# HongjianFang/DSurfTomo

Hardware: AMD Instinct MI355X
Metric: source-period FMM solves/sec on NxN grid; travel-time max-abs-err vs ref (higher is better)
Workload: dtype f32

## Files before the change

dsurftomo_amd/csrc/bundle_kernel.hip:

```cpp
#include "kernels.h"
#include "receiver_core.h"
#include "wave_ops.h"

namespace dsa {

namespace {

__device__ __forceinline__ unsigned bf2u(float f) { return __float_as_uint(f); }
__device__ __forceinline__ float bu2f(unsigned u) { return __uint_as_float(u); }

enum { BC_READY = 0, BC_READY_ODD, BC_TMIN, BC_THETA, BC_FREEZE, BC_HASH, BC_OVERFLOW, BC_CUR, BC_STALE, BC_STALEMIN, BC_SLOWN, BC_FARALL, BC_COUNT };
constexpr int kFarStrikes = 8;
constexpr int kBundleCycleRounds = 8;
constexpr float kStaleWindows = 16.0f;
constexpr int kStaleRounds = 6;

typedef __attribute__((address_space(1))) unsigned long long BGU64;
typedef __attribute__((address_space(1))) char BGChar;
typedef __attribute__((address_space(1))) float BGF32;
typedef __attribute__((address_space(1))) const float BGCF32;
typedef float __attribute__((ext_vector_type(4))) BV4;
typedef __attribute__((address_space(1))) BV4 BGV4;
typedef float __attribute__((ext_vector_type(2))) BV2;
template <int MPL> struct BMem;
template <> struct BMem<4> { typedef BV4 V; typedef __attribute__((address_space(1))) BV4 GV; };
template <> struct BMem<2> { typedef BV2 V; typedef __attribute__((address_space(1))) BV2 GV; };
// ... 17 lines not shown
template <int CH>
__device__ __forceinline__ unsigned node_or(unsigned v)
{
    if (CH >= 2) v |= (unsigned)__builtin_amdgcn_update_dpp(0, (int)v, 0xb1, 0xf, 0xf, false);
    if (CH >= 4) v |= (unsigned)__builtin_amdgcn_update_dpp(0, (int)v, 0x4e, 0xf, 0xf, false);
    if (CH >= 8) v |= (unsigned)__builtin_amdgcn_update_dpp(0, (int)v, 0x141, 0xf, 0xf, false);
    return v;
}

}

#ifdef DSA_BUNDLE_WAVES
#define DSA_BUNDLE_OCC(G, NT, MPL) __attribute__((amdgpu_waves_per_eu(DSA_BUNDLE_WAVES, DSA_BUNDLE_WAVES)))
#else
#define DSA_BUNDLE_OCC(G, NT, MPL) __attribute__((amdgpu_waves_per_eu((((NT) == 256 && ((MPL) == 2 || (G) == 16)) || (NT) == 768) ? 3 : 1, (((NT) == 256 && ((MPL) == 2 || (G) == 16)) || (NT) == 768) ? 3 : 2)))
#endif
template <int G, int NT, int MPL = 4, bool TIE = false>
__global__ __launch_bounds__(NT) DSA_BUNDLE_OCC(G, NT, MPL) void k_fim_bundle(const FimBundle* __restrict__ bundles, const FimProblem* __restrict__ problems,
                                                    const FimEnds* __restrict__ ends)
{
    constexpr int NW = NT / 64;
    constexpr int CH = G / MPL;
    typedef typename BMem<MPL>::V BV;
    typedef typename BMem<MPL>::GV BGV;
    constexpr int NPW = 64 / CH;
    constexpr unsigned GB = G * 4u * DSA_BSTRIDE;
    extern __shared__ unsigned dyn_lds[];
    __shared__ int sc[BC_COUNT];
    constexpr int kWaveBuf = 256, kTileBuf = NT > 256 ? 128 : 256, kClrWords = 4;
    __shared__ int wbuf[NW * kWaveBuf];
// ... 81 lines not shown
    BGChar* const Pb = (BGChar*)(Bslot + bd->p_offset);
    auto pv = [&](int id) -> float { return *(BGF32*)(Pb + ((unsigned)id << 2)); };

    __syncthreads();
    bool dead = false;
    {
        const BV4 inf4 = { kInf, kInf, kInf, kInf };
        for (int i = tid; i < ntile * (kTileRecs * G / 4) * DSA_BSTRIDE; i += NT) ((BGV4*)Bb)[i] = inf4;
        for (int i = tid; i < ntile * (kTileRecs / 4); i += NT) ((BGV4*)Pb)[i] = inf4;
        for (int i = tid; i < (1 << xlog); i += NT) *exc_at((unsigned)i) = kExcEmpty;
        for (int i = tid; i < (ntile << (kMaskShift - 3)); i += NT) *(BGU64*)(maskb + ((size_t)i << 3)) = 0ull;
        for (int i = tid; i < nwords; i += NT) tb[i] = 0u;
        if (tid == 0) {
            sc[BC_READY] = 0; sc[BC_READY_ODD] = 0; sc[BC_TMIN] = 0x7f800000; sc[BC_THETA] = 0x7f800000;
            sc[BC_FREEZE] = (int)0xff800000u; sc[BC_HASH] = 0; sc[BC_OVERFLOW] = 0; sc[BC_CUR] = 0; sc[BC_STALE] = (int)0xff800000u; sc[BC_STALEMIN] = 0x7f800000;
            sc[BC_SLOWN] = 0; sc[BC_FARALL] = bd->far_all ? 1 : 0;
            if (TIE && bd->cand) *(bd->cand + (size_t)my_slot * bd->cand_stride) = 0;
        }
        if (TIE && bd->cand) {
            BGV4* const seen4 = (BGV4*)(bd->cand + (size_t)my_slot * bd->cand_stride + ((bd->cand_cap + 4) & ~3));
            const BV4 zero4 = { 0.0f, 0.0f, 0.0f, 0.0f };
            for (int i = tid; i < kTieSeenSlots / 4; i += NT) seen4[i] = zero4;
        }
        __threadfence_block();
        __syncthreads();
        typedef __attribute__((address_space(1))) const Rec GCRec;
        for (int m = 0; m < nmem; ++m) {
            const FimEnds* const E = ends + s_member[m];
            const FimProblem* const pm = problems + s_member[m];
            const bool from_records = E->Fpin != nullptr;
            GCRec* const W = from_records ? (GCRec*)E->Fpin : (GCRec*)E->W;
// ... 60 lines not shown
        h.in[1] = ix + 1 < nnx;    h.in_outer[1] = ix + 2 < nnx;
        h.in[2] = iz > 0;          h.in_outer[2] = iz > 1;
        h.in[3] = iz + 1 < nnz;    h.in_outer[3] = iz + 2 < nnz;
        float val[9], tau[9];
        int kid[9];
#pragma unroll
        for (int q = 0; q < 4; ++q) {
            val[q] = h.in[q] ? *(BGF32*)(Bb + (unsigned)nid[q] * GB + mb) : kInf;
            val[4 + q] = h.in_outer[q] ? *(BGF32*)(Bb + (unsigned)nid[4 + q] * GB + mb) : kInf;
            kid[q] = nid[q]; kid[4 + q] = nid[4 + q];
        }
        val[8] = *(BGF32*)(Bb + (unsigned)id * GB + mb);
        kid[8] = id;
#pragma unroll
        for (int q = 0; q < 9; ++q) tau[q] = val[q];
#pragma nounroll
        for (int it = 0; it < 9; ++it) {
            float v = val[0], t = tau[0];
            if (__builtin_signbit(v)) { bool pin; t = exc_lookup(kid[0] * G + mo, &pin); v = pin ? v : -v; }
            const int k0 = kid[0];
#pragma unroll
            for (int j = 0; j < 8; ++j) { val[j] = val[j + 1]; tau[j] = tau[j + 1]; kid[j] = kid[j + 1]; }
            val[8] = v; tau[8] = t; kid[8] = k0;
        }
#pragma unroll
        for (int q = 0; q < 4; ++q) { h.near_[q] = val[q]; h.near_tau[q] = tau[q]; h.outer[q] = val[4 + q]; h.outer_tau[q] = tau[4 + q]; }
        *t_old = val[8]; *k_old = tau[8];
    };
    auto slow_member = [&](int id, int mo, int half, float stale, unsigned& evals, unsigned& nchanged, unsigned& hv_lane, float& kmin_lane, float& smin_lane) -> bool {
        if (mo >= nmem) return false;
// ... 61 lines not shown
        float t_old, k_old;
        load_hood(id, mo, ix, iz, h, &t_old, &k_old);
        if (t_pinned(t_old)) return;
        float k = kInf, ti = -1.0f;
        const float slown = *(BGCF32*)(slowb + (unsigned)id * npb + (unsigned)s_map[mo] * 4u);
        const NodeGeom geom = { p.ri, risti[ix], p.dnx, p.dnz };
        (void)solve_node_t<true>(h, slown, geom, &k, &ti);
        const FimProblem* const pm = problems + s_member[mo];
        if (ti >= 0.0f && pm->tie) {
            if (ti > 0.0f) { atomicAdd((unsigned*)pm->tie + 2, 1u); atomicAdd((unsigned*)pm->tie + 3, (unsigned)(fminf(ti, 1.0f) * (1.0f / kTieSumUnit))); }
            else atomicAdd((unsigned*)pm->tie + 5, 1u);
            if (ti > pm->tie_threshold) { atomicAdd((unsigned*)pm->tie, 1u); atomicMax((unsigned*)pm->tie + 1, bf2u(ti)); }
        }
    };
    int* const wq = slowq + wave * kSlowQ;
    int qn = 0;
    int cn = 0;
    int* const cand_g = (TIE && bd->cand && bd->cand_list) ? bd->cand + (size_t)my_slot * bd->cand_stride : nullptr;
    const bool listing = TIE && __builtin_amdgcn_readfirstlane(cand_g != nullptr ? 1 : 0) != 0;
    bool clost = false;
    auto cand_push = [&](bool on, int word) {
        const unsigned long long bal = __ballot(on);
        if (!bal) return;
        const int pos = cn + __popcll(bal & ((1ull << lane) - 1ull));
        cn += __popcll(bal);
        if (qn + cn >= kSlowQ - 1) { clost = true; return; }
        if (on) wq[kSlowQ - 1 - pos] = word;
    };
    auto cand_flush = [&]() {
        if (!cn || !cand_g) { cn = 0; clost = false; return; }
        int base = -1;
        if (lane == 0) {
            if (clost) (void)atomicMax(cand_g, bd->cand_cap + 1);
            else if (__hip_atomic_load(cand_g, __ATOMIC_RELAXED, __HIP_MEMORY_SCOPE_AGENT) <= bd->cand_cap) base = atomicAdd(cand_g, cn);
        }
        base = __builtin_amdgcn_readfirstlane(base);
        if (!clost && base >= 0) for (int i = lane; i < cn; i += 64) if (base + i < bd->cand_cap) cand_g[1 + base + i] = wq[kSlowQ - 1 - i];
        cn = 0; clost = false;
    };

    int rounds = 0, stall = 0, freezes = 0, sm_same = 0, far_strikes = 0;
    float sm_prev = kInf, sm_prev2 = kInf;
    unsigned hist[4] = { 1u, 2u, 3u, 4u };
    float best_tmin = -kInf;
    unsigned evals = 0, nchanged = 0;
    const int sub = lane % CH, nslot = lane / CH;
    const unsigned sub_b = (unsigned)sub * (4u * MPL);
    unsigned mp[MPL], vmask = 0u;
#pragma unroll
    for (int m = 0; m < MPL; ++m) { mp[m] = (unsigned)s_map[sub * MPL + m] * 4u; if (sub * MPL + m < nmem) vmask |= 1u << m; }
    bool sl_vec = (bd->np % MPL) == 0;
    {
        const int base = sub * MPL < nmem ? s_map[sub * MPL] : 0;
        sl_vec = sl_vec && (base % MPL) == 0 && base + MPL <= bd->np;
#pragma unroll
        for (int m = 1; m < MPL; ++m) if (sub * MPL + m < nmem && s_map[sub * MPL + m] != base + m) sl_vec = false;
        if (sl_vec) mp[0] = (unsigned)base * 4u;
    }
    sl_vec = __all(sl_vec);

#ifdef DSA_BUNDLE_CLOCKS
    unsigned long long bt[4] = { 0, 0, 0, 0 }, bt0 = wall_clock64();
#define DSA_BCLK(k) do { const unsigned long long t1_ = wall_clock64(); bt[k] += t1_ - bt0; bt0 = t1_; } while (0)
#else
#define DSA_BCLK(k) do { } while (0)
#endif
    for (; !dead;) {
        const float theta = bu2f((unsigned)sc[BC_THETA]);
        const bool open = !(theta < kInf);
        const float freeze = bu2f((unsigned)sc[BC_FREEZE]);
        const bool frozen_any = freeze > -kInf;
        const float stale = bu2f((unsigned)sc[BC_STALE]);
        const float far_margin = sc[BC_FARALL] ? kInf : far_margin0;

        int seen = 0;
        float tmin_lane = kInf;
        int* const nbuf = wbuf + wave * kWaveBuf;
        int* const tbuf = wtile + wave * kTileBuf;
        unsigned* const clr = wclr + wave * kTileBuf * kClrWords;
        constexpr int kQ = kTileBuf / 64, kI = kWaveBuf / 64;
// ... 150 lines not shown
                        if (idx >= tbase && idx < tbase + take) tbuf[ntw + idx - tbase] = (w << 5) + b2;
                        ++idx;
                    }
                    ntw += take; tbase += take;
                }
                if (ntw) { sweep_tiles(ntw); ntw = 0; }
            }
        }
        tmin_lane = wave_min(tmin_lane);
        if (lane == 0) {
            if (tmin_lane < kInf) atomicMin(reinterpret_cast<unsigned*>(&sc[BC_TMIN]), bf2u(tmin_lane));
            if (seen) atomicAdd(&sc[BC_CUR], seen);
        }
        __syncthreads();
        DSA_BCLK(0);
        const int cnt = sc[BC_CUR];
        if (cnt == 0) break;

        const int nready_even = sc[BC_READY] < rhalf ? sc[BC_READY] : rhalf;
        const int nready_odd = sc[BC_READY_ODD] < rhalf ? sc[BC_READY_ODD] : rhalf;
        unsigned hv_lane = 0u;
        float kmin_lane = kInf, smin_lane = kInf;
        for (int half = 0; half < 2; ++half) {
            const int nready = half ? nready_odd : nready_even;
            for (int j0 = wave * NPW; j0 < nready; j0 += NW * NPW) {
                const int j = j0 + nslot;
                const bool act = j < nready;
                const unsigned ent = act ? (unsigned)ready[half ? rhalf + j : j] : 0u;
                const int id = (int)(ent & ((1u << kFarShift) - 1u));
                const unsigned farc = ent >> kFarShift;
// ... 74 lines not shown
                __builtin_amdgcn_s_setprio(1);
                if (any_changed) {
                    *(BGV*)(Bb + (unsigned)id * GB + sub_b) = outv;
                    if (sub == 0) *(BGF32*)(Pb + ((unsigned)id << 2)) = outv[0];
                }
                bool any_slow = false;
#pragma unroll
                for (int m = 0; m < MPL; ++m) any_slow = any_slow | slowm[m];
                if (__any(any_slow)) {
                    bool again = false;
#pragma unroll
                    for (int m = 0; m < MPL; ++m) {
                        const bool push = slowm[m];
                        const unsigned long long bal = __ballot(push);
                        const int pos = qn + __popcll(bal & ((1ull << lane) - 1ull));
                        if (push && pos < kSlowQ - 1 - cn) wq[pos] = (id << 4) | (sub * MPL + m);
                        again = again || (push && pos >= kSlowQ - 1 - cn);
                        qn += __popcll(bal);
                    }
                    if (again) { atomicOr((unsigned long long*)(mask_at(id >> 6) + half), 1ull << (id & 63)); atomicOr(&tb[(id >> 6) >> 5], 1u << ((id >> 6) & 31)); }
                }
                if (listing) {
                    unsigned tiem = 0u;
#pragma unroll
                    for (int m = 0; m < MPL; ++m) {
                        const float v = outv[m];
                        const bool eq = (v == vn[0][m]) | (v == vn[1][m]) | (v == vn[2][m]) | (v == vn[3][m]);
                        tiem |= (eq & (v < kInf) & donem[m]) ? 1u << m : 0u;
                    }
                    if (__any(tiem != 0u)) {
#pragma nounroll
                        for (int m = 0; m < MPL; ++m) cand_push(((tiem >> m) & 1u) != 0u, (id << 4) | (sub * MPL + m));
                    }
                }
                unsigned wm = 0u;
#pragma unroll
                for (int q = 0; q < 4; ++q) wm |= (actn[q] ? 1u << q : 0u) | ((acto[q] & in_outer[q]) ? 16u << q : 0u);
                wm = node_or<CH>(wm);
                {
                    const unsigned chg = node_or<CH>(any_changed ? 1u : 0u);
                    const float pt = outv[0];
                    if (sub == 0 && chg && !__builtin_signbit(pt) && pt < stale) smin_lane = fminf(smin_lane, pt);
                }
                if (sub == 0 && wm) activate_node(id, wm, half);
            }
            if (lane == 0 && qn) atomicAdd(&sc[BC_SLOWN], qn);
            qn = qn < kSlowQ - 1 - cn ? qn : max(kSlowQ - 1 - cn, 0);
            for (int base = 0; base < qn; base += 64) {
                const int e = base + lane < qn ? wq[base + lane] : -1;
                bool tied = false;
                if (e >= 0) tied = slow_member(e >> 4, e & 15, half, stale, evals, nchanged, hv_lane, kmin_lane, smin_lane);
                if (listing) cand_push(tied, (int)((unsigned)e | kCandAlways));
            }
            qn = 0;
            if (TIE) cand_flush();
            if (half == 1) {
                const unsigned hv = wave_sum(hv_lane);
                const float kmin = wave_min(kmin_lane), smin = wave_min(smin_lane);
                if (lane == 0) {
                    if (hv) atomicAdd(reinterpret_cast<unsigned*>(&sc[BC_HASH]), hv);
                    if (kmin < kInf) atomicMin(reinterpret_cast<unsigned*>(&sc[BC_TMIN]), bf2u(kmin));
                    if (smin < kInf) atomicMin(reinterpret_cast<unsigned*>(&sc[BC_STALEMIN]), bf2u(smin));
                }
            }
            __syncthreads();
            DSA_BCLK(1 + half);
        }
        if (tid == 0) {
            {
                const int slown = sc[BC_SLOWN];
                sc[BC_SLOWN] = 0;
                if (!sc[BC_FARALL]) {
                    if (slown * 12 > (nready_even + nready_odd) * nmem && nready_even + nready_odd >= 64) { if (++far_strikes >= kFarStrikes) sc[BC_FARALL] = 1; }
                    else if (far_strikes > 0) --far_strikes;
                }
            }
            sc[BC_READY] = 0; sc[BC_READY_ODD] = 0; sc[BC_CUR] = 0;
            float tmin = bu2f((unsigned)sc[BC_TMIN]);
            {
                const float sm = bu2f((unsigned)sc[BC_STALEMIN]);
                sc[BC_STALEMIN] = 0x7f800000;
// ... 9 lines not shown
            sc[BC_STALE] = (int)bf2u(best_tmin - kStaleWindows * p.window);
            const bool repeat = hsh != 0u && (hsh == hist[1] || hsh == hist[2] || hsh == hist[3] || hsh == hist[0]);
            hist[3] = hist[2]; hist[2] = hist[1]; hist[1] = hist[0]; hist[0] = hsh;
            if (repeat) { if (++stall >= kBundleCycleRounds) { const float fz = (sm_same >= kStaleRounds ? sm_prev : best_tmin) + p.window;
                                                                 if (fz > bu2f((unsigned)sc[BC_FREEZE])) sc[BC_FREEZE] = (int)bf2u(fz); stall = 0; ++freezes; } }
            else stall = 0;
        }
        ++rounds;
        __syncthreads();
        DSA_BCLK(3);
        if (sc[BC_OVERFLOW]) break;
        if (rounds > p.max_rounds) { dead = true; break; }
    }
    const bool failed = rounds > p.max_rounds;
#ifdef DSA_BUNDLE_CLOCKS
    if (tid == 0 && p.clocks) { p.clocks[0] = bt[0]; p.clocks[1] = bt[1]; p.clocks[2] = bt[2]; p.clocks[3] = bt[3]; }
#endif

    {
        unsigned long long e64 = evals, c64 = nchanged;
        for (int o = 32; o > 0; o >>= 1) { e64 += __shfl_xor(e64, o); c64 += __shfl_xor(c64, o); }
        if (lane == 0) { atomicAdd(reinterpret_cast<unsigned long long*>(p.info + 4), e64); atomicAdd(reinterpret_cast<unsigned long long*>(p.info + 6), c64); }
    }
    __threadfence_block();
    __syncthreads();
    if (TIE && !failed && !sc[BC_OVERFLOW]) {
        constexpr int LPN = G / 4, NPI = 64 / LPN;
        const int csub = lane % LPN, cnode = lane / LPN;
        const BV4 inf4 = { kInf, kInf, kInf, kInf };
        int cq = 0;
        bool lost = false;
// ... 170 lines not shown
                    }
                }
            }
        }
        census_flush();
        if (lost && lane < nmem) {
            const FimProblem* const pm = problems + s_member[lane];
            if (pm->tie) { atomicAdd((unsigned*)pm->tie, 1u); atomicMax((unsigned*)pm->tie + 1, bf2u(kInf)); }
        }
        __syncthreads();
    }
    for (int m = 0; m < nmem; ++m) {
        const FimEnds* const E = ends + s_member[m];
        const FimProblem* const pm = problems + s_member[m];
        if (tid == 0) {
            pm->info[0] = rounds; pm->info[1] = 0; pm->info[3] = m == 0 ? freezes : 0;
            if (TIE && pm->tie) { pm->tie[4] = freezes; pm->tie[7] = cand_g ? __hip_atomic_load(cand_g, __ATOMIC_RELAXED, __HIP_MEMORY_SCOPE_AGENT) : -1; }
            if (failed && pm->info[2] != -2) pm->info[2] = -1;
            if (sc[BC_OVERFLOW]) pm->info[2] = -2;
        }
        if (E->rays) {
            const GridDesc g = E->g;
            for (int r = tid; r < E->nrays; r += NT) {
                const RayDesc rd = E->rays[r];
                if (!(rd.flags & kRayTime)) continue;
                float t;
                if (!receiver_time(g, E->scx, E->scz, rd, (const float*)Bslot + m, E->veln, E->dpl, &t, G * DSA_BSTRIDE)) atomicExch(E->err, E->ray0 + r + 1);
                E->out[rd.data] = t;
            }
        }
    }
// ... 111 lines not shown
```

dsurftomo_amd/csrc/engine.h:

```cpp
#pragma once

#include <hip/hip_runtime.h>

#include <string>
#include <vector>

#include "host_geometry.h"
#include "kernels.h"

namespace dsa {

template <class T>
struct DevBuf {
    T* p = nullptr;
    size_t cap = 0;
};

struct SpmvState;

constexpr int kDefaultExactTies = 1;
constexpr float kDefaultTieThreshold = 2.0e-5f;
constexpr float kDefaultTieSumThreshold = 0.0f;
constexpr int kDefaultTieCountThreshold = 0;
constexpr int kDefaultTieFrozenBundles = 0;
// ... 56 lines not shown
    int field_pool_opt = 0;
    size_t per_slot_bytes = 0;
    size_t plan_budget = 0;
    std::vector<int> h_launch_rank;
    int bundle_opt = 1;
    int ray_lanes_opt = 0;
    float bundle_window_opt = 0.0f;
    int bundle_G_now = 0;
    int bundle_threads_opt = 0;
    int bundle_max_rounds = 0;
    int bundle_mpl = 0;
    bool bundle_wide = false;
    int bundle_mpl_now = 4, bundle_mpl_b = 2;
    int bundle_threads_b = 256;
    int bundle_tail_opt = 1;
    int bundle_far_all = 0;
    int bundles_a = 0, bundles_b = 0, bundle_Gb = 0;
    hipStream_t stream2 = nullptr;
    hipEvent_t ev_b0 = nullptr, ev_b1 = nullptr;
    hipError_t make_stream2();
    int bundle_refined_opt = 1;
    bool refined_bundles_failed = false;
    bool refined_bundles_now = false;
    std::vector<FimBundle> h_bundles_r;
    DevBuf<FimBundle> bundles_r_d;
    DevBuf<FimEnds> ends_r;
    DevBuf<float> Br_pool, slowIr;
    DevBuf<unsigned long long> exc_br;
    DevBuf<int> lists_br, cand_br;
    size_t slowIr_off_b = 0;
// ... 156 lines not shown
```

dsurftomo_amd/csrc/engine.hip:

```cpp
#include <hip/hip_runtime.h>

#include <algorithm>
#include <chrono>
#include <cstdarg>
#include <cstdio>
#include <cstring>
#include <string>
#include <map>
#include <vector>

#include "../../include/dsurftomo_amd.h"
#include "engine.h"

namespace dsa {

static std::string g_create_error;

void Engine::fail(int code, const char* fmt, ...)
{
    char buf[512];
    va_list ap;
    va_start(ap, fmt);
    vsnprintf(buf, sizeof buf, fmt, ap);
    va_end(ap);
// ... 817 lines not shown
            stats[DSA_STAT_BUNDLES] += nbundles; stats[DSA_STAT_BUNDLED_UNITS] += n - nsolo;
            stats[DSA_STAT_FOOTPRINT_MB] = std::max(stats[DSA_STAT_FOOTPRINT_MB], ((double)pool_slots * (double)per_slot_bytes + (double)chunk * (double)per_unit_bytes) / 1.0e6 + bundle_mb);
        }
        for (int u = 0; u < n; ++u) {
            const int32_t* fi = &h_info[(size_t)u * 16];
            if (fi[10] == -3) { fail(DSA_ERR_INTERNAL, "unit %d: no free field slot within the wait bound (pool of %d slots, claimed by compare-and-swap: a pool smaller than the resident workgroups on very long solves, or corrupted busy flags; set option field_pool = -1 for a slot per unit)", first + u, pool_slots); return DSA_ERR_INTERNAL; }
            if (fi[2] < 0 || fi[10] == -1) { fail(DSA_ERR_INTERNAL, "unit %d: fixed-point solve did not converge (rounds %d/%d)", first + u, fi[0], fi[8]); return DSA_ERR_INTERNAL; }
            if (h_flags[(size_t)u * 4 + 1]) { fail(DSA_ERR_INTERNAL, "unit %d: serial march guard %d (1/17 window, 2/18 tree, 32 exception table)", first + u, h_flags[(size_t)u * 4 + 1]); return DSA_ERR_INTERNAL; }
            stats[DSA_STAT_ROUNDS_MAX] = std::max(stats[DSA_STAT_ROUNDS_MAX], (double)fi[8]);
            h_unit_rounds[(size_t)(first + u)] = fi[8];
            unsigned long long ev;
            std::memcpy(&ev, fi + 12, 8);
            stats[DSA_STAT_EVALS_TOTAL] += (double)ev;
            std::memcpy(&ev, fi + 14, 8);
            stats[DSA_STAT_CHANGES_TOTAL] += (double)ev;
            stats[DSA_STAT_RESCANS] += fi[1] + fi[9];
            stats[DSA_STAT_FREEZES] += fi[3] + fi[11];
        }
        if (!h_tie0.empty()) {
            const std::vector<char> fl = tie_verdicts(first, n, h_tie0.data(), h_info.data(), nbundles > 0);
            for (int u = 0; u < n; ++u) if (fl[(size_t)u]) { h_unit_flags[(size_t)(first + u)] |= 1; stats[DSA_STAT_TIE_UNITS] += 1.0; stats[DSA_STAT_TIE_UNITS_LEFT] += 1.0; }
        }
        for (int u = 0; u < n; ++u) stats[DSA_STAT_TIE_INFLUENCE_MAX] = std::max(stats[DSA_STAT_TIE_INFLUENCE_MAX], (double)h_unit_tie[(size_t)(first + u)]);
        last_chunk_first = first;
        last_chunk_n = n;
        fields_resident = n <= pool_slots && !marched_in_tiles;
        if (rows && trace_chunk(first, n, rw, iw, col, cap, nar) != 0) return status;
      } while (redo_chunk);
    }
    HIP_TRY(this, hipEventRecord(events[7], stream));
    HIP_TRY(this, hipEventSynchronize(events[7]));
// ... 188 lines not shown
    if (want_cand && ensure(cand_b, slots_total * cand_stride)) return status;
    if (ensure(B_pool, b_total) || ensure(exc_b, exc_total) || ensure(lists_b, slots_total * lists_c_stride) || ensure(bpool_gen, slots_total) ||
        ensure(bundles_d, (size_t)nb) || ensure(member_flag, (size_t)n) || ensure(slowI, (size_t)nmaps * nrec_c)) return status;
    if (!slowI_ready) { launch_interleave_maps(slow.p, nrec_c, nmaps, slowI.p, stream); slowI_ready = true; }
    h_bundles.assign((size_t)nb, FimBundle{});
    int rank = nsolo;
    for (int k = 0; k < nb; ++k) {
        const Group& r = gr[k < bundles_a ? 0 : 1];
        const std::vector<int>& mem = k < bundles_a ? pieces[(size_t)k].second : tail[(size_t)(k - bundles_a)].second;
        const int kk = k < bundles_a ? k : k - bundles_a;
        FimBundle& bd = h_bundles[(size_t)k];
        bd.B = B_pool.p + r.b_off; bd.b_stride = r.b_stride; bd.p_offset = (size_t)r.G * DSA_BSTRIDE * nrec_c;
        bd.exc = exc_b.p + r.exc_off; bd.exc_stride = (size_t)1 << r.xlog; bd.exc_log2cap = r.xlog;
        bd.lists = lists_b.p + r.slot0 * lists_c_stride; bd.lists_stride = lists_c_stride;
        bd.slot_busy = r.slots < r.count ? bpool_gen.p + r.slot0 : nullptr; bd.nslots = r.slots; bd.slot = r.slots < r.count ? 0 : kk;
        bd.slowI = slowI.p; bd.np = nmaps; bd.far_all = bundle_far_all;
        bd.cand = want_cand ? cand_b.p + r.slot0 * cand_stride : nullptr; bd.cand_stride = cand_stride; bd.cand_cap = (int)cand_cap; bd.cand_list = tie_list_opt;
        bd.nmem = (int)mem.size();
        for (int m = 0; m < kBundleMax; ++m) { bd.member[m] = 0; bd.map[m] = 0; }
        for (int m = 0; m < bd.nmem; ++m) {
            const int u = mem[(size_t)m];
            h_launch_rank[(size_t)u] = rank;
            bd.member[m] = rank++;
            bd.map[m] = h_src[(size_t)(first + u)].period;
        }
    }
    refined_bundles_now = bundle_refined_opt && (nb >= 128 || bundle_refined_opt == 2) && !refined_bundles_failed && exact_ties != 2;
    if (refined_bundles_now) {
        const size_t nrec_r = kRefRecs;
        const int xlog_r0 = exc_log2cap_of(kRefMax, kRefMax);
        const size_t lists_r_stride = ((size_t)kFimMaskInts * kRefTiles * kRefTiles + 2 + 1) & ~(size_t)1;
// ... 375 lines not shown
    if (n == "fim_sorted" && (value == 0 || value == 1)) { en->planned = false; en->fim_sorted = (int)value; return 0; }
    if (n == "ray_path_cap" && value >= 0 && value <= (1 << 24)) { en->ray_path_cap = (int)value; return 0; }
    if (n == "disp_group_shift" && value >= -1 && value <= 3) { en->disp_group_shift = (int)value; return 0; }
    if (n == "disp_layers_lds" && (value == -1 || value == 0 || value == 1)) { en->disp_layers_lds = (int)value; return 0; }
    if (n == "exc_log2cap" && (value == 0 || (value >= 6 && value <= 24))) { en->planned = false; en->exc_log2cap_opt = (int)value; return 0; }
    if (n == "rows_on_device" && (value == 0 || value == 1)) { en->rows_on_device = value != 0; return 0; }
    if (n == "lsmr_device_vectors" && (value == 0 || value == 1)) { en->lsmr_device_vectors = (int)value; return 0; }
    if (n == "field_pool" && value >= -1) { en->planned = false; en->field_pool_opt = (int)value; return 0; }
    if (n == "ray_lanes" && (value == 0 || value == 1 || value == 4)) { en->ray_lanes_opt = (int)value; return 0; }
    if (n == "bundle_window_cells" && value >= 0) { en->bundle_window_opt = (float)value; return 0; }
    if (n == "bundle_threads" && (value == 0 || value == 256 || value == 512 || value == 768)) { en->bundle_threads_opt = (int)value; return 0; }
    if (n == "bundle_max_rounds" && value >= 0) { en->bundle_max_rounds = (int)value; return 0; }
    if (n == "bundle_tail" && (value == 0 || value == 1)) { en->bundle_tail_opt = (int)value; return 0; }
    if (n == "bundle_refined" && (value == 0 || value == 1 || value == 2)) { en->bundle_refined_opt = (int)value; return 0; }
    if (n == "bundle_far_all" && (value == 0 || value == 1)) { en->bundle_far_all = (int)value; return 0; }
    if (n == "bundle_pool" && value >= 0) { en->bundle_pool_opt = (int)value; return 0; }
    if (n == "bundle_members_per_lane" && (value == 0 || value == 4 || value == 2)) { en->bundle_mpl = (int)value; return 0; }
    if (n == "bundle" && (value == 0 || value == 1 || value == 4 || value == 8 || value == 16)) { en->planned = false; en->bundle_opt = (int)value; return 0; }
    if (n == "exact_ties" && (value == 0 || value == 1 || value == 2)) { en->exact_ties = (int)value; return 0; }
    if (n == "tie_threshold" && value >= 0) { en->tie_threshold = (float)value; return 0; }
    if (n == "tie_detect" && (value == 0 || value == 1)) { en->tie_detect = (int)value; return 0; }
    if (n == "tie_sum_threshold" && value >= 0) { en->tie_sum_threshold = (float)value; return 0; }
    if (n == "tie_count_threshold" && value >= 0) { en->tie_count_threshold = (int)value; return 0; }
    if (n == "tie_frozen_bundles" && (value == 0 || value == 1)) { en->tie_frozen_bundles = (int)value; return 0; }
    if (n == "tie_map_strict" && (value == 0 || value == 1)) { en->tie_map_strict = (int)value; return 0; }
    if (n == "tie_scale_guard" && (value == 0 || value == 1)) { en->tie_scale_guard = (int)value; return 0; }
    if (n == "handoff_replay" && (value == 0 || value == 1)) { en->handoff_replay = (int)value; return 0; }
    if (n == "tie_tolerance" && value > 0) { en->tie_tolerance = (float)value; return 0; }
    if (n == "bundle_order" && (value == 0 || value == 1 || value == 2 || value == 3)) { en->bundle_order_opt = (int)value; return 0; }
    if (n == "tie_list" && (value == 0 || value == 1)) { en->tie_list_opt = (int)value; return 0; }
// ... 260 lines not shown
```

dsurftomo_amd/csrc/kernels.h:

```cpp
#pragma once

#include <hip/hip_runtime.h>
#include <stdint.h>

#include "source_stage.h"

namespace dsa {

struct RayDesc { int src; float rx, rz; float sin_rx; int data; int flags; };
constexpr int kRayTime = 1, kRayPath = 2;

constexpr int kClockSlots = 32;
constexpr int kTieWords = 16;
constexpr float kTieSumUnit = 0x1p-30f;
constexpr int kTieSeenLog2 = 14, kTieSeenSlots = 1 << kTieSeenLog2;

struct FimProblem {
    Rec* F;
    float* Tc;
    unsigned long long* exc;
    int exc_log2cap;
    const float* slow;
    const float* risti;
    const int* seed;
// ... 59 lines not shown
    unsigned long long* exc;
    size_t exc_stride;
    int exc_log2cap;
    int* lists;
    size_t lists_stride;
    size_t p_offset;
    int* slot_busy;
    int nslots, slot;
    const float* slowI;
    int np;
    int* cand;
    size_t cand_stride;
    int cand_cap;
    int cand_list;
    int far_all;
    int nmem;
    int member[kBundleMax];
    int map[kBundleMax];
};
size_t bundle_lds_bytes(int tile_words);
void launch_fim_bundles(const FimBundle* d_bundles, int nbundles, int G, int threads , const FimProblem* d_problems, const FimEnds* d_ends, int tile_words, hipStream_t stream,
                        int members_per_lane = 4 ,
                        bool tie = false );
void launch_interleave_maps(const float* d_slow_all, size_t field_stride, int np, float* d_slowI, hipStream_t stream);

size_t fim_lds_bytes(const FimLaunch& l);
void launch_fim(const FimProblem* d_problems, int nproblems, const FimLaunch& l, hipStream_t stream, const FimEnds* d_ends = nullptr);

void launch_gridder(const GridDesc& g, const float* d_velv, const float* d_basis, float* d_veln, float* d_slow,
                    hipStream_t stream);
// ... 100 lines not shown
```

dsurftomo_amd/csrc/stage_kernels.hip:

```cpp
#include "kernels.h"
#include "receiver_core.h"
#include "exact_march.h"

namespace dsa {

namespace {

__device__ __forceinline__ SourceScratch scratch_of(const BatchPtrs& b, int s)
{
    SourceScratch w;
    const size_t rr = (size_t)kRefMax * kRefMax;
    w.slow_r = b.slow_r + (size_t)s * kRefRecs;
    w.F_r = b.F_r + (size_t)s * kRefRecs;
    w.S_r = b.S_r + s * rr;
    w.risti_r = b.risti_r + (size_t)s * kRefMax;
    w.vcorner = b.vcorner + (size_t)s * 4;
    w.rst = b.rst + (size_t)s * kRWin * kRWin;
    w.cst = b.cst + (size_t)s * kCWinMax * kCWinMax;
    w.cinit = b.cinit + (size_t)s * kCWinMax * kCWinMax;
    w.heap = b.heap + (size_t)s * kHeapCap;
    w.flags = b.flags + (size_t)s * 4;
    return w;
}

// ... 394 lines not shown
                                const float* risti_c, float window_r, float window_c, FimProblem* prob_r,
                                FimProblem* prob_c, int32_t* info, unsigned long long* clocks, const int* __restrict__ launch_rank,
                                int32_t* tie, float tie_threshold, FimEnds* ends_c, const RayDesc* __restrict__ rays, const float* __restrict__ veln_all,
                                size_t veln_stride, float dpl, float* out, int32_t* err, const int* __restrict__ member_flag, float window_b, int max_rounds_b, float window_t, FimEnds* ends_r)
{
    const int s = blockIdx.x * blockDim.x + threadIdx.x;
    if (s >= nsrc) return;
    const SourceDesc sd = b.src[s];
    FimProblem r;
    r.Tc = nullptr; r.exc = nullptr; r.exc_log2cap = 0;
    r.F = b.F_r + (size_t)s * kRefRecs; r.slow = b.slow_r + (size_t)s * kRefRecs; r.risti = b.risti_r + (size_t)s * kRefMax;
    r.seed = b.seed_r + (size_t)s * kSeedR; r.seed_count = b.nseed_r + s; r.seed_cap = kSeedR; r.lists = b.lists + (size_t)s * b.lists_stride;
    r.nnx = sd.rnx; r.nnz = sd.rnz; r.nbx = sd.nbx_r; r.nbz = sd.nbz_r;
    r.ri = g.earth; r.dnx = sd.rdnx; r.dnz = sd.rdnz; r.window = window_r;
    r.max_rounds = 64 * (sd.rnx + sd.rnz) + 4096;
    r.clocks = nullptr;
    r.info = info + (size_t)s * 16;
    r.tie = tie ? tie + (size_t)s * kTieWords : nullptr; r.tie_threshold = tie_threshold;
    r.ended = b.flags + (size_t)s * 4;
    const int rank = launch_rank ? launch_rank[s] : s;
    if (ends_r) {
        prob_r[rank] = r;
        FimEnds er{};
        er.Fpin = r.F;
        ends_r[rank] = er;
    } else prob_r[s] = r;
    const bool recycled = b.pool < nsrc;
    const int slot = recycled ? rank % b.pool : s;
    const bool member = member_flag && member_flag[s];
    FimProblem c;
    c.F = nullptr;
// ... 67 lines not shown
```

dsurftomo_amd/engine.py:

```python
import ctypes as C
import os

import numpy as np

_HERE = os.path.dirname(os.path.abspath(__file__))
LIB_PATH = os.environ.get("DSA_LIB_PATH") or os.path.join(_HERE, "libdsurftomo_amd.so")

STAT_NAMES = ("ms_total", "ms_fim_coarse", "ms_fim_refined", "ms_stages", "launches_fim_coarse", "units",
              "rounds_max", "evals_total", "chunk", "rescans", "freezes", "rays", "ray_steps", "rays_clamped",
              "ms_rays", "ms_rows", "nar", "ms_dispersion", "curves", "changes_total", "tie_units", "exact_units", "exact_pops", "ms_exact", "field_slots", "footprint_mb", "bundle_size", "bundles", "bundled_units", "bundle_slots", "bundle_threads", "tie_units_left", "tie_influence_max", "exact_pool", "exact_tiles", "tie_units_strict", "tie_prone_maps", "tie_units_tied", "tie_units_by_scale", "handoffs_replayed")

_f32, _i32, _vp = C.c_float, C.c_int, C.c_void_p
_lib = None


class EngineError(RuntimeError):
    def __init__(self, code, text):
        super().__init__("dsurftomo_amd error %d: %s" % (code, text))
        self.code = code


def load_library():
    global _lib
    if _lib is not None:
        return _lib
# ... 408 lines not shown
```

include/dsurftomo_amd.h:

```cpp
#ifndef DSURFTOMO_AMD_H
#define DSURFTOMO_AMD_H

#include <stddef.h>
#include <stdint.h>

#ifdef __cplusplus
extern "C" {
#endif

typedef struct dsa_engine dsa_engine;

enum dsa_status {
    DSA_OK = 0,
    DSA_ERR_DEVICE = -1,
    DSA_ERR_ARGUMENT = -2,
    DSA_ERR_OUTSIDE = -3,
    DSA_ERR_INTERNAL = -4,
    DSA_ERR_STATE = -5,
    DSA_ERR_CAPACITY = -6
};

int dsa_create(dsa_engine** out, int device_index);
void dsa_destroy(dsa_engine* e);
const char* dsa_error_string(const dsa_engine* e);
// ... 96 lines not shown
       DSA_STAT_LAUNCHES_FIM_COARSE, DSA_STAT_UNITS, DSA_STAT_ROUNDS_MAX, DSA_STAT_EVALS_TOTAL,
       DSA_STAT_CHUNK, DSA_STAT_RESCANS, DSA_STAT_FREEZES, DSA_STAT_RAYS, DSA_STAT_RAY_STEPS,
       DSA_STAT_RAYS_CLAMPED, DSA_STAT_MS_RAYS, DSA_STAT_MS_ROWS, DSA_STAT_NAR, DSA_STAT_MS_DISPERSION,
       DSA_STAT_CURVES, DSA_STAT_CHANGES_TOTAL, DSA_STAT_TIE_UNITS, DSA_STAT_EXACT_UNITS, DSA_STAT_EXACT_POPS,
       DSA_STAT_MS_EXACT, DSA_STAT_FIELD_SLOTS, DSA_STAT_FOOTPRINT_MB, DSA_STAT_BUNDLE_SIZE, DSA_STAT_BUNDLES,
       DSA_STAT_BUNDLED_UNITS, DSA_STAT_BUNDLE_SLOTS, DSA_STAT_BUNDLE_THREADS,
       DSA_STAT_TIE_UNITS_LEFT,
       DSA_STAT_TIE_INFLUENCE_MAX,
       DSA_STAT_EXACT_POOL,
       DSA_STAT_EXACT_TILES,
       DSA_STAT_TIE_UNITS_STRICT,
       DSA_STAT_TIE_PRONE_MAPS,
       DSA_STAT_TIE_UNITS_TIED,
       DSA_STAT_TIE_UNITS_BY_SCALE,
       DSA_STAT_HANDOFFS_REPLAYED,
       DSA_STAT_COUNT };
int dsa_get_stats(const dsa_engine* e, double* out );

int dsa_calsurfg(const int* nx, const int* ny, const int* nz, const int* nparpi, const float* vels,
                 int* iw, float* rw, int* col, float* dsurf,
                 const float* goxdf, const float* gozdf, const float* dvxdf, const float* dvzdf,
                 const int* kmaxRc, const int* kmaxRg, const int* kmaxLc, const int* kmaxLg,
                 const double* tRc, const double* tRg, const double* tLc, const double* tLg,
                 const int* wavetype, const int* igrt, const int* periods, const float* depz,
                 const float* minthk, const float* scxf, const float* sczf, const float* rcxf,
                 const float* rczf, const int* nrc1, const int* nsrcsurf1, const int* kmax,
                 const int* nsrcsurf, const int* nrcf, int* nar);

int dsa_synthetic(const int* nx, const int* ny, const int* nz, const int* nparpi, const float* vels,
                  float* obst,
// ... 44 lines not shown
```

Before: 45180.

## Defer bundle slow-queue drain to second half and skip clean sign-fix pass

Slow-path members queued in the first half-sweep are now kept and drained once after the second half, always evaluated with half=1, so each round does one slow-queue pass instead of two. The neighbourhood loader skips its nine-step exception lookup loop when no lane sees a negative-flagged value. The change also adds a configurable slow-queue capacity, an optional cross-wave pooled drain (off by default), per-wave clock probes, and a queue-overflow counter that is split out of the rescan statistic. Deferring the drain changes when slow updates become visible, which can alter convergence and the number of rounds.

```diff
diff --git a/dsurftomo_amd/csrc/bundle_kernel.hip b/dsurftomo_amd/csrc/bundle_kernel.hip
--- a/dsurftomo_amd/csrc/bundle_kernel.hip
+++ b/dsurftomo_amd/csrc/bundle_kernel.hip
@@ -9,7 +9,7 @@
 __device__ __forceinline__ unsigned bf2u(float f) { return __float_as_uint(f); }
 __device__ __forceinline__ float bu2f(unsigned u) { return __uint_as_float(u); }
 
-enum { BC_READY = 0, BC_READY_ODD, BC_TMIN, BC_THETA, BC_FREEZE, BC_HASH, BC_OVERFLOW, BC_CUR, BC_STALE, BC_STALEMIN, BC_SLOWN, BC_FARALL, BC_COUNT };
+enum { BC_READY = 0, BC_READY_ODD, BC_TMIN, BC_THETA, BC_FREEZE, BC_HASH, BC_OVERFLOW, BC_CUR, BC_STALE, BC_STALEMIN, BC_SLOWN, BC_FARALL, BC_QFULL, BC_COUNT };
 constexpr int kFarStrikes = 8;
 constexpr int kBundleCycleRounds = 8;
 constexpr float kStaleWindows = 16.0f;
@@ -57,6 +57,12 @@
 #define DSA_BUNDLE_OCC(G, NT, MPL) __attribute__((amdgpu_waves_per_eu(DSA_BUNDLE_WAVES, DSA_BUNDLE_WAVES)))
 #else
 #define DSA_BUNDLE_OCC(G, NT, MPL) __attribute__((amdgpu_waves_per_eu((((NT) == 256 && ((MPL) == 2 || (G) == 16)) || (NT) == 768) ? 3 : 1, (((NT) == 256 && ((MPL) == 2 || (G) == 16)) || (NT) == 768) ? 3 : 2)))
+#endif
+#ifndef DSA_BUNDLE_POOL
+#define DSA_BUNDLE_POOL 0
+#endif
+#ifndef DSA_BUNDLE_SLOW_EVERY_HALF
+#define DSA_BUNDLE_SLOW_EVERY_HALF 0
 #endif
 template <int G, int NT, int MPL = 4, bool TIE = false>
 __global__ __launch_bounds__(NT) DSA_BUNDLE_OCC(G, NT, MPL) void k_fim_bundle(const FimBundle* __restrict__ bundles, const FimProblem* __restrict__ problems,
@@ -168,7 +174,7 @@
         if (tid == 0) {
             sc[BC_READY] = 0; sc[BC_READY_ODD] = 0; sc[BC_TMIN] = 0x7f800000; sc[BC_THETA] = 0x7f800000;
             sc[BC_FREEZE] = (int)0xff800000u; sc[BC_HASH] = 0; sc[BC_OVERFLOW] = 0; sc[BC_CUR] = 0; sc[BC_STALE] = (int)0xff800000u; sc[BC_STALEMIN] = 0x7f800000;
-            sc[BC_SLOWN] = 0; sc[BC_FARALL] = bd->far_all ? 1 : 0;
+            sc[BC_SLOWN] = 0; sc[BC_FARALL] = bd->far_all ? 1 : 0; sc[BC_QFULL] = 0;
             if (TIE && bd->cand) *(bd->cand + (size_t)my_slot * bd->cand_stride) = 0;
         }
         if (TIE && bd->cand) {
@@ -259,6 +265,10 @@
         kid[8] = id;
 #pragma unroll
         for (int q = 0; q < 9; ++q) tau[q] = val[q];
+        unsigned sgn = 0u;
+#pragma unroll
+        for (int q = 0; q < 9; ++q) sgn |= bf2u(val[q]);
+        if (__any((int)sgn < 0))
 #pragma nounroll
         for (int it = 0; it < 9; ++it) {
             float v = val[0], t = tau[0];
@@ -350,7 +360,8 @@
         }
     };
     int* const wq = slowq + wave * kSlowQ;
-    int qn = 0;
+    const int qcap = __builtin_amdgcn_readfirstlane(bd->slow_cap > 0 && bd->slow_cap < kSlowQ ? bd->slow_cap : kSlowQ);
+    int qn = 0, qn_kept = 0, slow_round = 0;
     int cn = 0;
     int* const cand_g = (TIE && bd->cand && bd->cand_list) ? bd->cand + (size_t)my_slot * bd->cand_stride : nullptr;
     const bool listing = TIE && __builtin_amdgcn_readfirstlane(cand_g != nullptr ? 1 : 0) != 0;
@@ -360,8 +371,8 @@
         if (!bal) return;
         const int pos = cn + __popcll(bal & ((1ull << lane) - 1ull));
         cn += __popcll(bal);
-        if (qn + cn >= kSlowQ - 1) { clost = true; return; }
-        if (on) wq[kSlowQ - 1 - pos] = word;
+        if (qn + cn >= qcap - 1) { clost = true; return; }
+        if (on) wq[qcap - 1 - pos] = word;
     };
     auto cand_flush = [&]() {
         if (!cn || !cand_g) { cn = 0; clost = false; return; }
@@ -371,7 +382,7 @@
             else if (__hip_atomic_load(cand_g, __ATOMIC_RELAXED, __HIP_MEMORY_SCOPE_AGENT) <= bd->cand_cap) base = atomicAdd(cand_g, cn);
         }
         base = __builtin_amdgcn_readfirstlane(base);
-        if (!clost && base >= 0) for (int i = lane; i < cn; i += 64) if (base + i < bd->cand_cap) cand_g[1 + base + i] = wq[kSlowQ - 1 - i];
+        if (!clost && base >= 0) for (int i = lane; i < cn; i += 64) if (base + i < bd->cand_cap) cand_g[1 + base + i] = wq[qcap - 1 - i];
         cn = 0; clost = false;
     };
 
@@ -398,8 +409,23 @@
 #ifdef DSA_BUNDLE_CLOCKS
     unsigned long long bt[4] = { 0, 0, 0, 0 }, bt0 = wall_clock64();
 #define DSA_BCLK(k) do { const unsigned long long t1_ = wall_clock64(); bt[k] += t1_ - bt0; bt0 = t1_; } while (0)
+    __shared__ unsigned long long s_wclk[2][NW][3];
+    unsigned long long wsum[8] = { 0, 0, 0, 0, 0, 0, 0, 0 }, wcnt[3] = { 0, 0, 0 }, half_t0 = bt0;
+#define DSA_BHALF0() do { half_t0 = bt0; } while (0)
+#define DSA_BWCLK(h, k) do { if (lane == 0) s_wclk[h][wave][k] = wall_clock64(); } while (0)
+#define DSA_BWCNT(i, v) do { wcnt[i] += (unsigned long long)(v); } while (0)
+#define DSA_BWCLK_SUM(h) do { if (tid == 0) { int wl_ = 0; for (int w_ = 1; w_ < NW; ++w_) if (s_wclk[h][w_][2] > s_wclk[h][wl_][2]) wl_ = w_; \
+        wsum[4 * (h) + 0] += s_wclk[h][wl_][0] - half_t0; wsum[4 * (h) + 1] += s_wclk[h][wl_][((h) || DSA_BUNDLE_SLOW_EVERY_HALF) ? 1 : 0] - s_wclk[h][wl_][0]; \
+        wsum[4 * (h) + 2] += s_wclk[h][wl_][2] - s_wclk[h][wl_][((h) || DSA_BUNDLE_SLOW_EVERY_HALF) ? 1 : 0]; wsum[4 * (h) + 3] += bt0 - s_wclk[h][wl_][2]; } half_t0 = bt0; } while (0)
 #else
 #define DSA_BCLK(k) do { } while (0)
+#define DSA_BWCLK(h, k) do { } while (0)
+#define DSA_BWCNT(i, v) do { } while (0)
+#define DSA_BWCLK_SUM(h) do { } while (0)
+#define DSA_BHALF0() do { } while (0)
+#endif
+#if DSA_BUNDLE_POOL
+    __shared__ int s_qn[NW];
 #endif
     for (; !dead;) {
         const float theta = bu2f((unsigned)sc[BC_THETA]);
@@ -580,6 +606,7 @@
         }
         __syncthreads();
         DSA_BCLK(0);
+        DSA_BHALF0();
         const int cnt = sc[BC_CUR];
         if (cnt == 0) break;
 
@@ -684,11 +711,11 @@
                         const bool push = slowm[m];
                         const unsigned long long bal = __ballot(push);
                         const int pos = qn + __popcll(bal & ((1ull << lane) - 1ull));
-                        if (push && pos < kSlowQ - 1 - cn) wq[pos] = (id << 4) | (sub * MPL + m);
-                        again = again || (push && pos >= kSlowQ - 1 - cn);
+                        if (push && pos < qcap - 1 - cn) wq[pos] = (id << 4) | (sub * MPL + m);
+                        again = again || (push && pos >= qcap - 1 - cn);
                         qn += __popcll(bal);
                     }
-                    if (again) { atomicOr((unsigned long long*)(mask_at(id >> 6) + half), 1ull << (id & 63)); atomicOr(&tb[(id >> 6) >> 5], 1u << ((id >> 6) & 31)); }
+                    if (again) { atomicOr((unsigned long long*)(mask_at(id >> 6) + half), 1ull << (id & 63)); atomicOr(&tb[(id >> 6) >> 5], 1u << ((id >> 6) & 31)); atomicAdd(&sc[BC_QFULL], 1); }
                 }
                 if (listing) {
                     unsigned tiem = 0u;
@@ -714,27 +741,51 @@
                 }
                 if (sub == 0 && wm) activate_node(id, wm, half);
             }
-            if (lane == 0 && qn) atomicAdd(&sc[BC_SLOWN], qn);
-            qn = qn < kSlowQ - 1 - cn ? qn : max(kSlowQ - 1 - cn, 0);
-            for (int base = 0; base < qn; base += 64) {
-                const int e = base + lane < qn ? wq[base + lane] : -1;
-                bool tied = false;
-                if (e >= 0) tied = slow_member(e >> 4, e & 15, half, stale, evals, nchanged, hv_lane, kmin_lane, smin_lane);
-                if (listing) cand_push(tied, (int)((unsigned)e | kCandAlways));
-            }
-            qn = 0;
-            if (TIE) cand_flush();
-            if (half == 1) {
-                const unsigned hv = wave_sum(hv_lane);
-                const float kmin = wave_min(kmin_lane), smin = wave_min(smin_lane);
-                if (lane == 0) {
-                    if (hv) atomicAdd(reinterpret_cast<unsigned*>(&sc[BC_HASH]), hv);
-                    if (kmin < kInf) atomicMin(reinterpret_cast<unsigned*>(&sc[BC_TMIN]), bf2u(kmin));
-                    if (smin < kInf) atomicMin(reinterpret_cast<unsigned*>(&sc[BC_STALEMIN]), bf2u(smin));
-                }
-            }
+            slow_round += qn - qn_kept;
+            if (qn > qcap - 1 - cn) qn = max(qcap - 1 - cn, 0);
+            qn_kept = qn;
+            DSA_BWCLK(half, 0);
+            if (half == 1 || DSA_BUNDLE_SLOW_EVERY_HALF) {
+                if (lane == 0 && slow_round) atomicAdd(&sc[BC_SLOWN], slow_round);
+#if DSA_BUNDLE_POOL
+                if (lane == 0) s_qn[wave] = qn;
+                __syncthreads();
+                int qtot = 0;
+#pragma unroll
+                for (int w = 0; w < NW; ++w) qtot += s_qn[w];
+                for (int base = wave * 64; base < qtot; base += NW * 64) {
+                    int k = base + lane, e = -1;
+                    if (k < qtot) {
+                        int w = 0;
+                        while (k >= s_qn[w]) { k -= s_qn[w]; ++w; }
+                        e = slowq[w * kSlowQ + k];
+                    }
+#else
+                for (int base = 0; base < qn; base += 64) {
+                    const int e = base + lane < qn ? wq[base + lane] : -1;
+#endif
+                    bool tied = false;
+                    DSA_BWCNT(0, __popcll(__ballot(e >= 0))); DSA_BWCNT(1, 1);
+                    if (e >= 0) tied = slow_member(e >> 4, e & 15, DSA_BUNDLE_SLOW_EVERY_HALF ? half : 1, stale, evals, nchanged, hv_lane, kmin_lane, smin_lane);
+                    if (listing) cand_push(tied, (int)((unsigned)e | kCandAlways));
+                }
+                qn = 0; qn_kept = 0; slow_round = 0;
+                DSA_BWCLK(half, 1);
+                if (TIE) { DSA_BWCNT(2, cn && cand_g ? 1 : 0); cand_flush(); }
+                if (half == 1) {
+                    const unsigned hv = wave_sum(hv_lane);
+                    const float kmin = wave_min(kmin_lane), smin = wave_min(smin_lane);
+                    if (lane == 0) {
+                        if (hv) atomicAdd(reinterpret_cast<unsigned*>(&sc[BC_HASH]), hv);
+                        if (kmin < kInf) atomicMin(reinterpret_cast<unsigned*>(&sc[BC_TMIN]), bf2u(kmin));
+                        if (smin < kInf) atomicMin(reinterpret_cast<unsigned*>(&sc[BC_STALEMIN]), bf2u(smin));
+                    }
+                }
+            }
+            DSA_BWCLK(half, 2);
             __syncthreads();
             DSA_BCLK(1 + half);
+            DSA_BWCLK_SUM(half);
         }
         if (tid == 0) {
             {
@@ -774,7 +825,9 @@
     }
     const bool failed = rounds > p.max_rounds;
 #ifdef DSA_BUNDLE_CLOCKS
-    if (tid == 0 && p.clocks) { p.clocks[0] = bt[0]; p.clocks[1] = bt[1]; p.clocks[2] = bt[2]; p.clocks[3] = bt[3]; }
+    const int cb = ends[bd->member[0]].Fpin ? 20 : 8;
+    if (tid == 0 && p.clocks) { p.clocks[0] = bt[0]; p.clocks[1] = bt[1]; p.clocks[2] = bt[2]; p.clocks[3] = bt[3]; for (int q = 0; q < 8; ++q) p.clocks[cb + q] = wsum[q]; p.clocks[cb + 11] = (unsigned long long)rounds; }
+    if (lane == 0 && p.clocks) for (int q = 0; q < 3; ++q) if (wcnt[q]) atomicAdd(p.clocks + cb + 8 + q, wcnt[q]);
 #endif
 
     {
@@ -975,7 +1028,8 @@
         const FimEnds* const E = ends + s_member[m];
         const FimProblem* const pm = problems + s_member[m];
         if (tid == 0) {
-            pm->info[0] = rounds; pm->info[1] = 0; pm->info[3] = m == 0 ? freezes : 0;
+            pm->info[0] = rounds; pm->info[1] = m == 0 ? sc[BC_QFULL] : 0;
+            pm->info[3] = m == 0 ? freezes : 0;
             if (TIE && pm->tie) { pm->tie[4] = freezes; pm->tie[7] = cand_g ? __hip_atomic_load(cand_g, __ATOMIC_RELAXED, __HIP_MEMORY_SCOPE_AGENT) : -1; }
             if (failed && pm->info[2] != -2) pm->info[2] = -1;
             if (sc[BC_OVERFLOW]) pm->info[2] = -2;
diff --git a/dsurftomo_amd/csrc/engine.h b/dsurftomo_amd/csrc/engine.h
--- a/dsurftomo_amd/csrc/engine.h
+++ b/dsurftomo_amd/csrc/engine.h
@@ -94,6 +94,7 @@
     int bundle_mpl_now = 4, bundle_mpl_b = 2;
     int bundle_threads_b = 256;
     int bundle_tail_opt = 1;
+    int bundle_slow_queue = 0;
     int bundle_far_all = 0;
     int bundles_a = 0, bundles_b = 0, bundle_Gb = 0;
     hipStream_t stream2 = nullptr;
diff --git a/dsurftomo_amd/csrc/engine.hip b/dsurftomo_amd/csrc/engine.hip
--- a/dsurftomo_amd/csrc/engine.hip
+++ b/dsurftomo_amd/csrc/engine.hip
@@ -855,7 +855,12 @@
             stats[DSA_STAT_EVALS_TOTAL] += (double)ev;
             std::memcpy(&ev, fi + 14, 8);
             stats[DSA_STAT_CHANGES_TOTAL] += (double)ev;
-            stats[DSA_STAT_RESCANS] += fi[1] + fi[9];
+            {
+                const bool member = nbundles > 0 && h_member_flag[(size_t)u] != 0;
+                const int ovf = (member && refined_b ? fi[1] : 0) + (member ? fi[9] : 0);
+                stats[DSA_STAT_BUNDLE_QUEUE_OVERFLOWS] += (double)ovf;
+                stats[DSA_STAT_RESCANS] += fi[1] + fi[9] - ovf;
+            }
             stats[DSA_STAT_FREEZES] += fi[3] + fi[11];
         }
         if (!h_tie0.empty()) {
@@ -1074,7 +1079,7 @@
         bd.exc = exc_b.p + r.exc_off; bd.exc_stride = (size_t)1 << r.xlog; bd.exc_log2cap = r.xlog;
         bd.lists = lists_b.p + r.slot0 * lists_c_stride; bd.lists_stride = lists_c_stride;
         bd.slot_busy = r.slots < r.count ? bpool_gen.p + r.slot0 : nullptr; bd.nslots = r.slots; bd.slot = r.slots < r.count ? 0 : kk;
-        bd.slowI = slowI.p; bd.np = nmaps; bd.far_all = bundle_far_all;
+        bd.slowI = slowI.p; bd.np = nmaps; bd.far_all = bundle_far_all; bd.slow_cap = bundle_slow_queue;
         bd.cand = want_cand ? cand_b.p + r.slot0 * cand_stride : nullptr; bd.cand_stride = cand_stride; bd.cand_cap = (int)cand_cap; bd.cand_list = tie_list_opt;
         bd.nmem = (int)mem.size();
         for (int m = 0; m < kBundleMax; ++m) { bd.member[m] = 0; bd.map[m] = 0; }
@@ -1480,6 +1485,7 @@
     if (n == "bundle_tail" && (value == 0 || value == 1)) { en->bundle_tail_opt = (int)value; return 0; }
     if (n == "bundle_refined" && (value == 0 || value == 1 || value == 2)) { en->bundle_refined_opt = (int)value; return 0; }
     if (n == "bundle_far_all" && (value == 0 || value == 1)) { en->bundle_far_all = (int)value; return 0; }
+    if (n == "bundle_slow_queue" && (value == 0 || (value >= 257 && value <= 1024))) { en->planned = false; en->bundle_slow_queue = (int)value; return 0; }
     if (n == "bundle_pool" && value >= 0) { en->bundle_pool_opt = (int)value; return 0; }
     if (n == "bundle_members_per_lane" && (value == 0 || value == 4 || value == 2)) { en->bundle_mpl = (int)value; return 0; }
     if (n == "bundle" && (value == 0 || value == 1 || value == 4 || value == 8 || value == 16)) { en->planned = false; en->bundle_opt = (int)value; return 0; }
diff --git a/dsurftomo_amd/csrc/kernels.h b/dsurftomo_amd/csrc/kernels.h
--- a/dsurftomo_amd/csrc/kernels.h
+++ b/dsurftomo_amd/csrc/kernels.h
@@ -97,6 +97,7 @@
     int cand_cap;
     int cand_list;
     int far_all;
+    int slow_cap;
     int nmem;
     int member[kBundleMax];
     int map[kBundleMax];
diff --git a/dsurftomo_amd/csrc/stage_kernels.hip b/dsurftomo_amd/csrc/stage_kernels.hip
--- a/dsurftomo_amd/csrc/stage_kernels.hip
+++ b/dsurftomo_amd/csrc/stage_kernels.hip
@@ -432,7 +432,11 @@
     r.nnx = sd.rnx; r.nnz = sd.rnz; r.nbx = sd.nbx_r; r.nbz = sd.nbz_r;
     r.ri = g.earth; r.dnx = sd.rdnx; r.dnz = sd.rdnz; r.window = window_r;
     r.max_rounds = 64 * (sd.rnx + sd.rnz) + 4096;
+#ifdef DSA_BUNDLE_CLOCKS
+    r.clocks = clocks ? clocks + (size_t)s * kClockSlots : nullptr;
+#else
     r.clocks = nullptr;
+#endif
     r.info = info + (size_t)s * 16;
     r.tie = tie ? tie + (size_t)s * kTieWords : nullptr; r.tie_threshold = tie_threshold;
     r.ended = b.flags + (size_t)s * 4;
diff --git a/dsurftomo_amd/engine.py b/dsurftomo_amd/engine.py
--- a/dsurftomo_amd/engine.py
+++ b/dsurftomo_amd/engine.py
@@ -8,7 +8,7 @@
 
 STAT_NAMES = ("ms_total", "ms_fim_coarse", "ms_fim_refined", "ms_stages", "launches_fim_coarse", "units",
               "rounds_max", "evals_total", "chunk", "rescans", "freezes", "rays", "ray_steps", "rays_clamped",
-              "ms_rays", "ms_rows", "nar", "ms_dispersion", "curves", "changes_total", "tie_units", "exact_units", "exact_pops", "ms_exact", "field_slots", "footprint_mb", "bundle_size", "bundles", "bundled_units", "bundle_slots", "bundle_threads", "tie_units_left", "tie_influence_max", "exact_pool", "exact_tiles", "tie_units_strict", "tie_prone_maps", "tie_units_tied", "tie_units_by_scale", "handoffs_replayed")
+              "ms_rays", "ms_rows", "nar", "ms_dispersion", "curves", "changes_total", "tie_units", "exact_units", "exact_pops", "ms_exact", "field_slots", "footprint_mb", "bundle_size", "bundles", "bundled_units", "bundle_slots", "bundle_threads", "tie_units_left", "tie_influence_max", "exact_pool", "exact_tiles", "tie_units_strict", "tie_prone_maps", "tie_units_tied", "tie_units_by_scale", "handoffs_replayed", "bundle_queue_overflows")
 
 _f32, _i32, _vp = C.c_float, C.c_int, C.c_void_p
 _lib = None
diff --git a/include/dsurftomo_amd.h b/include/dsurftomo_amd.h
--- a/include/dsurftomo_amd.h
+++ b/include/dsurftomo_amd.h
@@ -134,6 +134,7 @@
        DSA_STAT_TIE_UNITS_TIED,
        DSA_STAT_TIE_UNITS_BY_SCALE,
        DSA_STAT_HANDOFFS_REPLAYED,
+       DSA_STAT_BUNDLE_QUEUE_OVERFLOWS,
        DSA_STAT_COUNT };
 int dsa_get_stats(const dsa_engine* e, double* out );
 
```

After: 45880, median of 4. +1.5%, better.
